# robotseu/ORB_Line_SLAM

Measured on AMD Instinct MI355X. Metric: stereo frames/s extract+match (ORB+LBD), KITTI 1242x375, higher is better.
Workload: dtype u8; 1 GPU; C3: 1242x375 stereo, 2000 ORB + 500 LBD per image, extract + stereo point/line match + f2f LBD match + SearchByBoW vs the previous frame (synthetic k=10 L=6 vocabulary, ComputeBoW included); parallelism=frame-sharded x1, distinct_pairs=512, order=shuffled, scene=default

## Files before the change

orb_line_slam_amd/csrc/api.cpp:

```cpp
#include "ctx.hpp"
#include "staging.hpp"
#include <map>
#include <mutex>

namespace olf {
static thread_local std::string g_err;
void set_error(const std::string& s) { g_err = s; }

int check_device(const olf_ctx* c, const char* who)
{
    int d = -1;
    if (hipGetDevice(&d) != hipSuccess || d != c->device) { set_error(std::string(who) + ": the context belongs to another device than the current one"); return OLF_ERR_INVALID; }
    return OLF_OK;
}

static int check_landscape(const olf_ctx* c, const char* who)
{
    if (c->orb.portrait) {
        set_error(std::string(who) + ": the context's image is portrait (a pyramid level's octree would have round(width / height) == 0 root cells, where the "
                                     "reference divides by zero): no detector runs in it");
        return OLF_ERR_INVALID;
    }
    return OLF_OK;
}
// ... 150 lines not shown
const char* olf_last_error(void) { return g_err.c_str(); }

int olf_device_count(void)
{
    int n = 0;
    if (hipGetDeviceCount(&n) != hipSuccess) return 0;
    return n;
}

int olf_default_params(olf_params* p)
{
    if (!p) return OLF_ERR_INVALID;
    std::memset(p, 0, sizeof(*p));
    p->abi_version = OLF_ABI_VERSION; p->struct_size = (uint32_t)sizeof(olf_params);
    p->orb.nfeatures = 2000; p->orb.scale_factor = 1.2f; p->orb.nlevels = 8; p->orb.ini_th_fast = 20; p->orb.min_th_fast = 7;
    p->line.lsd_nfeatures = 500; p->line.min_line_length = 0.025; p->line.lsd_refine = 0; p->line.lsd_scale = 1.2;
    p->line.lsd_sigma_scale = 0.6; p->line.lsd_quant = 2.0; p->line.lsd_ang_th = 22.5; p->line.lsd_log_eps = 1.0;
    p->line.lsd_density_th = 0.6; p->line.lsd_n_bins = 1024;
    p->line.conv_seed_order = 1;
    p->stereo.fx = 718.856f; p->stereo.bf = 386.1448f; p->stereo.matching_s_ws = 10; p->stereo.line_sim_th = 0.75;
    p->stereo.min_ratio_12_l = 0.9; p->stereo.min_disp = 1.0; p->stereo.line_horiz_th = 0.1; p->stereo.stereo_overlap_th = 0.75;
    p->stereo.ls_min_disp_ratio = 0.7; p->stereo.best_lr_matches = 1;
    return OLF_OK;
}

void olf_ctx_destroy(olf_ctx* c)
{
    if (!c) return;
    if (c->has_tables) angle_tables_release(c->device, c->params.line.conv_libm_float);
    if (c->h_outslab) (void)hipHostFree(c->h_outslab);
    for (void* p : c->allocs) (void)hipFree(p);
    for (void* p : c->scratch) if (p) (void)hipFree(p);
    for (auto& r : c->prof_recs) { (void)hipEventDestroy(r.a); (void)hipEventDestroy(r.b); }
    for (hipEvent_t e : c->prof_pool) (void)hipEventDestroy(e);
    if (c->ev_fork) (void)hipEventDestroy(c->ev_fork);
    if (c->ev_front) (void)hipEventDestroy(c->ev_front);
    if (c->ev_sort) (void)hipEventDestroy(c->ev_sort);
    if (c->ev_lbd) (void)hipEventDestroy(c->ev_lbd);
    if (c->ev_join) (void)hipEventDestroy(c->ev_join);
    if (c->stream2) (void)hipStreamDestroy(c->stream2);
    if (c->stream) (void)hipStreamDestroy(c->stream);
    delete c;
}

int olf_ctx_create(const olf_params* p, int width, int height, int max_images, olf_ctx** out)
{
    if (!p || !out || width < 64 || height < 64 || max_images < 1) { set_error("olf_ctx_create: bad argument"); return OLF_ERR_INVALID; }
    *out = nullptr;
    if (p->abi_version != OLF_ABI_VERSION || p->struct_size != (uint32_t)sizeof(olf_params)) {
        set_error("olf_ctx_create: the parameter block was not initialised by this library's olf_default_params() (abi_version / struct_size differ: "
                  "caller built against another include/orbline_types.h)");
        return OLF_ERR_INVALID;
    }
    int ndev = 0;
    if (hipGetDeviceCount(&ndev) != hipSuccess || ndev < 1) {
        set_error("olf_ctx_create: no HIP device visible (this library has no CPU path)");
        return OLF_ERR_NODEVICE;
    }
    olf_ctx* c = new olf_ctx();
    c->params = *p; c->W = width; c->H = height; c->max_images = max_images;
    int rc = c->orb.build(p->orb, width, height);
    if (rc != OLF_OK) {
        set_error(rc == OLF_ERR_CAPACITY ? "olf_ctx_create: more than 32760 key points on one pyramid level (nfeatures too large for this scale factor / level count)"
                  : (width > kMaxOrbSide || height > kMaxOrbSide) ? "olf_ctx_create: image wider or higher than 4131 pixels (FAST candidates are packed with 12 bits per coordinate)"
                                         : "olf_ctx_create: image size / ORB parameters not supported (every pyramid level needs at least 62 x 62 pixels)");
        delete c; return rc;
    }
    auto fail = [&](int code) { olf_ctx_destroy(c); return code; };
    if (hipGetDevice(&c->device) != hipSuccess) return fail(OLF_ERR_HIP);
    if (hipDeviceGetAttribute(&c->limits.nCU, hipDeviceAttributeMultiprocessorCount, c->device) != hipSuccess || c->limits.nCU <= 0) c->limits.nCU = 64;
    if (hipDeviceGetAttribute(&c->limits.maxLds, hipDeviceAttributeMaxSharedMemoryPerBlock, c->device) != hipSuccess) c->limits.maxLds = 64 * 1024;
    if (hipStreamCreateWithFlags(&c->stream, hipStreamNonBlocking) != hipSuccess) { set_error("hipStreamCreate failed"); return fail(OLF_ERR_HIP); }
    const OrbGeom& g = c->orb.geom;
    const size_t n = (size_t)max_images;
    OrbDeviceBufs& b = c->ob;
    const bool allocTrace = getenv("OLF_ALLOC_TRACE") != nullptr;
#define A(ptr, count) do { if ((rc = dev_alloc(c, &(ptr), (count))) != OLF_OK) return fail(rc); \
                           if (allocTrace) fprintf(stderr, "alloc %-18s %8.3f MB per image\n", #ptr, (double)(count) * sizeof(*(ptr)) / 1e6 / (double)n); } while (0)
    A(b.pyr, n * g.pyrBytes); A(b.blur, n * g.pyrBytes);
    A(b.cells, n * g.totalCells * g.cellCap); A(b.cellCount, n * g.totalCells);
    A(b.cand, n * g.candTotal); A(b.candNode, n * g.candTotal); A(b.candCount, n * g.nlevels);
    if (g.maxNodes > 2048) A(b.octSpill, n * g.nlevels * octree_lds_bytes(g.maxNodes));
    A(b.lvlKp, n * g.kpTotal); A(b.lvlCount, n * g.nlevels); A(b.lvlAngle, n * g.kpTotal);
    A(b.rx, c->orb.rx.size() + 1); A(b.ry, c->orb.ry.size() + 1); A(b.geom, 1); A(b.status, 256);
    A(c->d_sad, ((n + 1) / 2) * g.outCap); A(c->d_bestkey, ((n + 1) / 2) * g.outCap); A(c->d_rowperm, n * g.outCap);
    A(c->d_images, n * width * height);
#undef A
    if (hipMemcpy(b.rx, c->orb.rx.data(), c->orb.rx.size() * sizeof(ResizeCoef), hipMemcpyHostToDevice) != hipSuccess ||
        hipMemcpy(b.ry, c->orb.ry.data(), c->orb.ry.size() * sizeof(ResizeCoef), hipMemcpyHostToDevice) != hipSuccess ||
        hipMemcpy(b.geom, &g, sizeof(OrbGeom), hipMemcpyHostToDevice) != hipSuccess ||
        hipMemset(b.status, 0, 1024) != hipSuccess) {
        set_error("olf_ctx_create: table upload failed");
        return fail(OLF_ERR_HIP);
    }
    rc = c->line.build(p->line, width, height, max_images);
    if (rc != OLF_OK) { set_error("olf_ctx_create: LSD parameters not supported"); return fail(rc); }
    LineGeom& lg = c->line.geom;
    int prLeast = 0, prGreatest = 0;
    (void)hipDeviceGetStreamPriorityRange(&prLeast, &prGreatest);
    if (hipStreamCreateWithPriority(&c->stream2, hipStreamNonBlocking, prLeast) != hipSuccess ||
        hipEventCreateWithFlags(&c->ev_fork, hipEventDisableTiming) != hipSuccess || hipEventCreateWithFlags(&c->ev_front, hipEventDisableTiming) != hipSuccess || hipEventCreateWithFlags(&c->ev_sort, hipEventDisableTiming) != hipSuccess ||
        hipEventCreateWithFlags(&c->ev_lbd, hipEventDisableTiming) != hipSuccess ||
        hipEventCreateWithFlags(&c->ev_join, hipEventDisableTiming) != hipSuccess) { set_error("stream/event creation failed"); return fail(OLF_ERR_HIP); }
    LineDeviceBufs& l = c->lb;
#define A(ptr, count) do { if ((rc = dev_alloc(c, &(ptr), (count))) != OLF_OK) return fail(rc); \
                           if (allocTrace) fprintf(stderr, "alloc %-18s %8.3f MB per image\n", #ptr, (double)(count) * sizeof(*(ptr)) / 1e6 / (double)n); } while (0)
    const bool batchCtx = n > (size_t)kBatchCtxImages;
    const size_t keyWords = lg.wide ? 2 : 1;
    A(l.grad, n * lg.Ps); A(l.keysA, n * lg.Ps * keyWords); A(l.keysB, n * lg.Ps * keyWords);
    if (batchCtx && lg.Ps * 4 >= lg.pitchW * lg.H && lg.Ps * 4 >= lg.pitchS * lg.Hs) { l.lsdBlur = reinterpret_cast<uint8_t*>(l.keysA); l.scaled = reinterpret_cast<uint8_t*>(l.keysB); c->scaled_aliased = true; }
    else { A(l.lsdBlur, n * lg.pitchW * lg.H); A(l.scaled, n * lg.pitchS * lg.Hs); }
    A(l.topBuf, n * (size_t)lsd_seedsort_top_words()); A(l.keyCount, n * 32); A(l.maxN, n * 32); A(l.chunkCnt, n * ((lg.Ps + 4095) / 4096)); A(l.sortHist, n * (size_t)lsd_sort_max_chunks(lg.Ps) * 32); A(l.sortBase, n * 32);
    l.nChunks = lg.regionStride / 32;
    A(l.region, n * (size_t)lg.regionStride); l.ownerImages = (batchCtx || lg.wide) ? 0 : (int)std::min<size_t>(n, kMwMaxImages); A(l.owner, (size_t)l.ownerImages * lg.Ps); A(l.links, n * (size_t)l.nChunks);
    lg.logCap = lg.regionStride / 2;
    lg.spillBlocks = lg.regionStride / 2 >= lg.Ps ? 0 : (int)std::max<size_t>(4, n / 16);
    if (lg.spillBlocks) A(lg.spillArena, (size_t)lg.spillBlocks * 2 * lg.Ps);
    A(lg.spillCtl, 64); A(lg.spillOf, n);
    l.mgImages = (int)std::min<size_t>(n, kMgMaxImages); l.mgStride = lsd_grow_mg_stride(lg.maxRegions);
    A(l.mg, (size_t)l.mgImages * l.mgStride);
    A(l.rawLines, n * lg.maxDetect); A(l.rawCount, n); A(l.regCount, n); A(l.growFmt, n); A(l.lbdBlur, n * lg.pitchW * lg.H); A(l.dxdy, n * lg.pitchD * lg.H);
    A(l.rowSums, n * lg.outCap * 63 * 4); A(l.lbdStarts, n * lg.outCap * 64 * 2); A(l.rx, c->line.rx.size()); A(l.ry, c->line.ry.size()); A(l.geom, 1);
    A(c->d_ldist, ((n + 1) / 2) * lg.outCap * lg.outCap); A(c->d_lm21, ((n + 1) / 2) * lg.outCap);
    if (hipMalloc(&c->d_lprep, stereo_lines_prep_bytes((int)n, lg.outCap)) != hipSuccess) { set_error("hipMalloc failed"); return fail(OLF_ERR_HIP); }
    c->allocs.push_back(c->d_lprep);
    const bool slab = n <= 16;
    if (slab) {
        size_t off = 0;
        for (int k = 0; k < FB_FIELDS; ++k) { c->outslab_off[k] = off; off += (fb_bytes(c, k, n) + 255) & ~(size_t)255; }
        c->outslab_bytes = off;
        A(c->d_outslab, off);
        if (hipHostMalloc(reinterpret_cast<void**>(&c->h_outslab), off, hipHostMallocDefault) != hipSuccess) { set_error("hipHostMalloc failed"); return fail(OLF_ERR_HIP); }
    }
    for (int k = 0; k < FB_FIELDS; ++k) {
        uint8_t* q = nullptr;
        if (slab) q = c->d_outslab + c->outslab_off[k];
        else if ((rc = dev_alloc(c, &q, fb_bytes(c, k, n))) != OLF_OK) return fail(rc);
        fb_set_field(c->d_out, k, q);
        if (allocTrace) fprintf(stderr, "alloc %-18s %8.3f MB per image\n", kFrameFields[k].name, (double)fb_bytes(c, k, n) / 1e6 / (double)n);
    }
#undef A
    l.status = b.status;
    if (hipMemcpy(l.rx, c->line.rx.data(), c->line.rx.size() * sizeof(ResizeCoef), hipMemcpyHostToDevice) != hipSuccess ||
        hipMemcpy(l.ry, c->line.ry.data(), c->line.ry.size() * sizeof(ResizeCoef), hipMemcpyHostToDevice) != hipSuccess ||
        hipMemcpy(l.geom, &lg, sizeof(LineGeom), hipMemcpyHostToDevice) != hipSuccess) { set_error("line table upload failed"); return fail(OLF_ERR_HIP); }
    if ((rc = angle_tables_acquire(c->device, p->line.conv_libm_float, l, c->stream)) != OLF_OK) return fail(rc);
    c->has_tables = true;
    *out = c;
    return OLF_OK;
}

int olf_ctx_synchronize(olf_ctx* c)
{
    if (!c) return OLF_ERR_INVALID;
    OLF_HIP_CHECK(hipStreamSynchronize(c->stream));
    OLF_HIP_CHECK(hipStreamSynchronize(c->stream2));
    c->join_pending = false;
    return check_status(c);
}

int olf_ctx_set_input_event(olf_ctx* c, void* hip_event)
{
    if (!c) return OLF_ERR_INVALID;
    c->input_event = static_cast<hipEvent_t>(hip_event);
    return OLF_OK;
}

int olf_ctx_poll_status(olf_ctx* c)
{
    if (!c) return OLF_ERR_INVALID;
    return check_status(c);
}

// ... 359 lines not shown
```

orb_line_slam_amd/csrc/host_tables.cpp:

```cpp
#include "olf_internal.hpp"
#include "line_internal.hpp"
#include <algorithm>
#include <cmath>
#include <cfenv>

namespace olf {

static inline int cv_round_f(float v) { return (int)lrintf(v); }
static inline int cv_round_d(double v) { return (int)lrint(v); }
static inline int cv_floor(double v) { int i = (int)v; return i - (i > v); }
static inline int cv_ceil(double v) { int i = (int)v; return i + (i < v); }

std::vector<int> gaussian_taps_q8(int n, double sigma, int sum256)
{
    if (sum256) {
        std::vector<double> k(n);
        double s = 0;
        const double scale2X = -0.5 / (sigma * sigma);
        for (int i = 0; i < n; ++i) { const double x = i - (n - 1) * 0.5; k[i] = std::exp(scale2X * x * x); s += k[i]; }
        std::vector<int> q(n);
        double err = 0;
        int sum = 0;
        for (int i = 0; i < n / 2; ++i) {
            const double adj = k[i] / s * 256.0 + err;
            const int v = cv_round_d(adj);
            err = adj - v;
            q[i] = q[n - 1 - i] = v;
            sum += v;
        }
        q[n / 2] = 256 - 2 * sum;
        return q;
    }
    std::vector<float> cf(n);
    double scale2X = -0.5 / (sigma * sigma), sum = 0;
    for (int i = 0; i < n; ++i) {
        double x = i - (n - 1) * 0.5;
        cf[i] = (float)std::exp(scale2X * x * x);
        sum += cf[i];
    }
    sum = 1. / sum;
    std::vector<int> q(n);
    for (int i = 0; i < n; ++i) {
        cf[i] = (float)(cf[i] * sum);
        q[i] = cv_round_d((double)cf[i] * 256.0);
    }
    return q;
}

void resize_axis_coefs(int sn, int dn, double scale, bool clamp_like_x, ResizeCoef* coef)
{
    for (int d = 0; d < dn; ++d) {
        float f = (float)((d + 0.5) * scale - 0.5);
        int s = cv_floor(f);
        f -= s;
        if (clamp_like_x) {
            if (s < 0) { f = 0; s = 0; }
            if (s >= sn - 1) { f = 0; s = sn - 1; }
        }
        int a0 = cv_round_f((1.f - f) * 2048.f), a1 = cv_round_f(f * 2048.f);
        coef[d].ofs = (int16_t)s;
        coef[d].a0 = (int16_t)std::min(std::max(a0, -32768), 32767);
        coef[d].a1 = (int16_t)std::min(std::max(a1, -32768), 32767);
        coef[d].pad = 0;
    }
}

void resize_axis_coefs_exact(int sn, int dn, double scale, ResizeCoef* coef)
{
    for (int d = 0; d < dn; ++d) {
        const double f = scale * (d + 0.5) - 0.5;
        int i = cv_floor(f);
        int a = cv_round_d((f - i) * 256.0);
        if (i < 0) { i = 0; a = 0; }
        if (i >= sn - 1) { i = sn - 1; a = 0; }
        coef[d].ofs = (int16_t)i; coef[d].a0 = (int16_t)(256 - a); coef[d].a1 = (int16_t)a; coef[d].pad = 0;
    }
}

int OrbHostTables::build(const olf_orb_params& p, int W, int H)
{
    const int nlevels = p.nlevels;
    if (nlevels < 1 || nlevels > OLF_MAX_LEVELS || p.nfeatures < 1 || !(p.scale_factor > 1.0f)) return OLF_ERR_INVALID;
    if (W > kMaxOrbSide || H > kMaxOrbSide) return OLF_ERR_INVALID;
    const double scaleFactor = p.scale_factor;
    sf.assign(nlevels, 1.f); sigma2.assign(nlevels, 1.f); inv_sf.resize(nlevels); inv_sigma2.resize(nlevels);
    for (int i = 1; i < nlevels; ++i) {
        sf[i] = (float)(sf[i - 1] * scaleFactor);
        sigma2[i] = sf[i] * sf[i];
    }
    for (int i = 0; i < nlevels; ++i) {
        inv_sf[i] = 1.0f / sf[i];
        inv_sigma2[i] = 1.0f / sigma2[i];
    }
    nPerLevel.resize(nlevels);
    float factor = (float)(1.0f / scaleFactor);
    float nDesired = p.nfeatures * (1 - factor) / (1 - (float)std::pow((double)factor, (double)nlevels));
    int sum = 0;
    for (int l = 0; l < nlevels - 1; ++l) {
        nPerLevel[l] = cv_round_f(nDesired);
        sum += nPerLevel[l];
        nDesired *= factor;
    }
    nPerLevel[nlevels - 1] = std::max(p.nfeatures - sum, 0);

    OrbGeom& g = geom;
    g = OrbGeom();
    g.nlevels = nlevels; g.W = W; g.H = H; g.in_pitch = W;
    g.iniTh = std::min(std::max(p.ini_th_fast, 1), 255);
    g.minTh = std::min(std::max(p.min_th_fast, 1), 255);
    g.minTh = std::min(g.minTh, g.iniTh);
    {
        int v, v0, vmax = cv_floor(kHalfPatch * std::sqrt(2.f) / 2 + 1);
        int vmin = cv_ceil(kHalfPatch * std::sqrt(2.f) / 2);
        const double hp2 = kHalfPatch * kHalfPatch;
        for (v = 0; v <= vmax; ++v) g.umax[v] = cv_round_d(std::sqrt(hp2 - v * v));
        for (v = kHalfPatch, v0 = 0; v >= vmin; --v) {
            while (g.umax[v0] == g.umax[v0 + 1]) ++v0;
            g.umax[v] = v0;
            ++v0;
        }
    }
    std::vector<int> taps = gaussian_taps_q8(7, 2.0, p.conv_gauss_sum256);
    for (int i = 0; i < 7; ++i) g.blurTaps[i] = taps[i];

    rx.clear(); ry.clear();
    int off = 0, cells = 0, cand = 0, kps = 0, cellCap = 1, maxQuota = 1, maxKp = 1;
    for (int l = 0; l < nlevels; ++l) {
        LevelGeom& L = g.lv[l];
        L.w = cv_round_f((float)W * inv_sf[l]);
        L.h = cv_round_f((float)H * inv_sf[l]);
        if (L.w - 2 * kMinBorder < 30 || L.h - 2 * kMinBorder < 30) return OLF_ERR_INVALID;
        L.pitch = (L.w + 63) & ~63;
        L.offset = off;
        off += L.pitch * L.h;
        off = (off + 255) & ~255;
        L.maxBorderX = L.w - kMinBorder; L.maxBorderY = L.h - kMinBorder;
        const float width = (float)(L.maxBorderX - kMinBorder), height = (float)(L.maxBorderY - kMinBorder);
        L.nCols = (int)(width / 30.f); L.nRows = (int)(height / 30.f);
        L.wCell = (int)std::ceil(width / L.nCols); L.hCell = (int)std::ceil(height / L.nRows);
        L.wCellM = (uint32_t)(((1u << 20) + L.wCell - 1) / L.wCell); L.hCellM = (uint32_t)(((1u << 20) + L.hCell - 1) / L.hCell);
        if (L.w >= (1 << 14) || L.h >= (1 << 14) || L.wCell > 64 || L.hCell > 64) { L.wCellM = 0; L.hCellM = 0; }
        L.cellBase = cells;
        cells += L.nCols * L.nRows;
        cellCap = std::max(cellCap, ((L.wCell + 1) / 2) * ((L.hCell + 1) / 2));
        L.quota = nPerLevel[l];
        maxQuota = std::max(maxQuota, L.quota);
        L.nIni = (int)std::round(width / height);
        if (L.nIni < 1) { portrait = true; L.nIni = 1; }
        L.hX = width / L.nIni;
        L.scale = sf[l]; L.inv_scale = inv_sf[l];
        L.patch_size = (int)(31 * sf[l]);
        L.kpBase = kps; L.kpCap = std::max(L.quota + 8, 4 * L.nIni + 4); kps += L.kpCap;
        maxKp = std::max(maxKp, L.kpCap);
        if (l > 0) {
            const LevelGeom& P = g.lv[l - 1];
            L.resizeTabX = (int)rx.size(); L.resizeTabY = (int)ry.size();
            rx.resize(rx.size() + L.w); ry.resize(ry.size() + L.h);
            double inv_x = (double)L.w / P.w, inv_y = (double)L.h / P.h;
            resize_axis_coefs(P.w, L.w, 1. / inv_x, true, &rx[L.resizeTabX]);
            resize_axis_coefs(P.h, L.h, 1. / inv_y, false, &ry[L.resizeTabY]);
            L.resizeTiled = resize_tiled_fits(&rx[L.resizeTabX], &ry[L.resizeTabY], P.w, P.h, L.w, L.h) ? 1 : 0;
            if (L.resizeTiled && resize_strip_fits(&rx[L.resizeTabX], P.w, L.w)) L.resizeTiled |= 2;
        }
    }
    g.pyrBytes = off;
    g.totalCells = cells;
    g.cellCap = cellCap;
    if (cellCap > 1024) return OLF_ERR_CAPACITY;
    for (int l = 0; l < nlevels; ++l) {
        LevelGeom& L = g.lv[l];
        long cap = (long)L.nCols * L.nRows * cellCap;
        L.candCap = (int)std::min<long>(cap, 65535);
        L.candBase = cand;
        cand += (L.candCap + 63) & ~63;
    }
    g.candTotal = cand;
    g.kpTotal = kps;
    g.outCap = kps;
    int mn = 64;
    while (mn < maxKp) mn <<= 1;
    g.maxNodes = mn;
    if (mn > 32768) return OLF_ERR_CAPACITY;
    return OLF_OK;
}

int LineHostTables::build(const olf_line_params& p, int W, int H, int max_images)
{
    LineGeom& g = geom;
    g = LineGeom();
    if (p.lsd_refine < 0 || p.lsd_refine > 2) return OLF_ERR_INVALID;
    if (p.conv_seed_order != 0 && p.conv_seed_order != 1) return OLF_ERR_INVALID;
    if (p.conv_libm_float != 0 && p.conv_libm_float != 1) return OLF_ERR_INVALID;
    if (!(p.lsd_scale > 0) || p.lsd_n_bins < 2 || p.lsd_n_bins > (1 << 24) || !(p.lsd_ang_th > 0 && p.lsd_ang_th < 180)) return OLF_ERR_INVALID;
    const double kPI = 3.1415926535897932384626433832795;
    g.W = W; g.H = H; g.pitchW = (W + 63) & ~63; g.pitchD = (W + 3) & ~3;
    g.scale = p.lsd_scale;
    g.Ws = cv_round_d(W * p.lsd_scale); g.Hs = cv_round_d(H * p.lsd_scale);
    g.pitchS = (g.Ws + 63) & ~63;
    g.Ps = g.Ws * g.Hs;
    {
        int k = 0; while ((1 << k) < g.Ws) ++k;
        const int p = std::max(32, 22 + k);
// ... 87 lines not shown
```

orb_line_slam_amd/csrc/olf_internal.hpp:

```cpp
#pragma once
#include <hip/hip_runtime.h>
#include <stdint.h>
#include <string>
#include <vector>
#include "../../include/orbline_types.h"
#include "device_math.hpp"

#define OLF_HIP_CHECK(expr)                                                                 \
    do {                                                                                    \
        hipError_t _e = (expr);                                                             \
        if (_e != hipSuccess) {                                                             \
            olf::set_error(std::string(#expr) + ": " + hipGetErrorString(_e));              \
            return OLF_ERR_HIP;                                                             \
        }                                                                                   \
    } while (0)

#define OLF_TRY(expr)                  \
    do {                               \
        int _rc = (expr);              \
        if (_rc != OLF_OK) return _rc; \
    } while (0)

struct olf_ctx;

// ... 50 lines not shown
}
OLF_HD void csr_row(const int* __restrict__ offs, int n, int k, int& b, int& e) { const int last = offs[n]; csr_clamp(offs, k, last > 0 ? last : 0, b, e); }

OLF_HD int live_item(int v, int n_items, const uint8_t* __restrict__ bad, int* __restrict__ status, int bit)
{
    if (v >= n_items) { status_raise(status, bit); return -1; }
    return v < 0 || bad[v] ? -1 : v;
}

#ifdef __HIPCC__
__device__ __forceinline__ bool pair_in_batch(int f1, int f2, int n_frames) { return f1 >= 0 && f1 < n_frames && f2 >= 0 && f2 < n_frames && f1 != f2; }

__device__ __forceinline__ int wave_sum_i32(int v)
{
    v += __builtin_amdgcn_mov_dpp(v, 0xB1, 0xf, 0xf, true);
    v += __builtin_amdgcn_mov_dpp(v, 0x4E, 0xf, 0xf, true);
    v += __builtin_amdgcn_mov_dpp(v, 0x141, 0xf, 0xf, true);
    v += __builtin_amdgcn_mov_dpp(v, 0x140, 0xf, 0xf, true);
    return __builtin_amdgcn_readlane(v, 0) + __builtin_amdgcn_readlane(v, 16) + __builtin_amdgcn_readlane(v, 32) + __builtin_amdgcn_readlane(v, 48);
}

__device__ __forceinline__ int wave_min_i32(int v)
{
    v = min(v, __builtin_amdgcn_update_dpp(v, v, 0xB1, 0xf, 0xf, false));
    v = min(v, __builtin_amdgcn_update_dpp(v, v, 0x4E, 0xf, 0xf, false));
    v = min(v, __builtin_amdgcn_update_dpp(v, v, 0x141, 0xf, 0xf, false));
    v = min(v, __builtin_amdgcn_update_dpp(v, v, 0x140, 0xf, 0xf, false));
    return min(min(__builtin_amdgcn_readlane(v, 0), __builtin_amdgcn_readlane(v, 16)), min(__builtin_amdgcn_readlane(v, 32), __builtin_amdgcn_readlane(v, 48)));
}
__device__ __forceinline__ unsigned long long wave_vote(bool p) { return __builtin_amdgcn_ballot_w64(p); }
__device__ __forceinline__ int wave_rank_below(unsigned long long m) { return (int)__builtin_amdgcn_mbcnt_hi((unsigned)(m >> 32), __builtin_amdgcn_mbcnt_lo((unsigned)m, 0u)); }
__device__ __forceinline__ bool wave_bit(unsigned long long m) { return __builtin_amdgcn_inverse_ballot_w64(m); }
#endif

constexpr int kEdge = 19;
constexpr int kMinBorder = 16;
constexpr int kHalfPatch = 15;
constexpr int kMaxOrbSide = 4095 + 2 * kMinBorder + 4;
static_assert(kMaxOrbSide == 4131, "olf_ctx_create's message and include/orbline.h state this limit");

struct LevelGeom {
    int w, h, pitch;
    int offset;
    int maxBorderX, maxBorderY;
    int nCols, nRows, wCell, hCell;
    uint32_t wCellM, hCellM;
    int cellBase;
    int quota;
    int nIni;
    float hX;
    float scale;
    float inv_scale;
    int patch_size;
    int candBase;
    int candCap;
    int kpBase, kpCap;
    int resizeTabX, resizeTabY;
    int resizeTiled;
};

struct ResizeCoef { int16_t ofs; int16_t a0; int16_t a1; int16_t pad; };

struct OrbGeom {
    int nlevels;
    int W, H, in_pitch;
    int pyrBytes;
    int totalCells;
    int cellCap;
    int candTotal;
    int kpTotal;
    int outCap;
    int iniTh, minTh;
    int maxNodes;
    LevelGeom lv[OLF_MAX_LEVELS];
    int umax[16];
    int blurTaps[7];
};

struct OrbHostTables {
    std::vector<float> sf, inv_sf, sigma2, inv_sigma2;
    std::vector<int> nPerLevel;
    OrbGeom geom;
    std::vector<ResizeCoef> rx, ry;
    bool portrait = false;
    int build(const olf_orb_params& p, int W, int H);
};

std::vector<int> gaussian_taps_q8(int n, double sigma, int sum256 = 0);
void resize_axis_coefs(int sn, int dn, double scale, bool clamp_like_x, ResizeCoef* coef);

struct OrbDeviceBufs {
    uint8_t* pyr = nullptr;
    uint8_t* blur = nullptr;
    uint32_t* cells = nullptr;
    int* cellCount = nullptr;
    uint32_t* cand = nullptr;
    uint16_t* candNode = nullptr;
    int* candCount = nullptr;
    uint32_t* lvlKp = nullptr;
    int* lvlCount = nullptr;
    float* lvlAngle = nullptr;
    ResizeCoef* rx = nullptr;
    ResizeCoef* ry = nullptr;
    OrbGeom* geom = nullptr;
    int* status = nullptr;
    unsigned char* octSpill = nullptr;
};

int launch_orb_pyramid(const OrbGeom& g, const OrbDeviceBufs& b, const uint8_t* d_in, int n_images, hipStream_t s);
int launch_orb_fast(const OrbGeom& g, const OrbDeviceBufs& b, int n_images, hipStream_t s);
int launch_orb_octree(const OrbGeom& g, const OrbDeviceBufs& b, int n_images, hipStream_t s);
size_t octree_lds_bytes(int M);
int launch_orb_blur(const OrbGeom& g, const OrbDeviceBufs& b, int n_images, hipStream_t s);
int launch_orb_describe(const OrbGeom& g, const OrbDeviceBufs& b, int n_images, olf_keypoint* d_kps, uint8_t* d_desc,
                        int* d_counts, int out_cap, hipStream_t s);

struct Taps7 { int t[7]; };
int launch_sep7(const uint8_t* src, size_t srcImgStride, int srcPitch, uint8_t* dst, size_t dstImgStride, int dstPitch, int W, int H,
                const int* taps7, int n_images, hipStream_t s);
int launch_sep_wide(const uint8_t* src, size_t srcImgStride, int srcPitch, uint8_t* dst, size_t dstImgStride, int dstPitch, int W, int H,
                    const int* taps, int r, int n_images, hipStream_t s);

bool resize_tiled_fits(const ResizeCoef* rx, const ResizeCoef* ry, int sw, int sh, int dw, int dh);
bool resize_strip_fits(const ResizeCoef* rx, int sw, int dw, int ncols = 4);
int launch_resize_tiled(const uint8_t* src, size_t srcImgStride, int srcPitch, int sw, int sh, uint8_t* dst, size_t dstImgStride, int dstPitch,
                        int dw, int dh, const ResizeCoef* d_rx, const ResizeCoef* d_ry, int n_images, hipStream_t s, bool strip = false);

int launch_cvt_gray(const uint8_t* src, uint8_t* dst, int w, int h, int code, int n_images, hipStream_t s);
int launch_init_rectify_map(const double* ir9, const double* k8, double fx, double fy, double u0, double v0, int w, int h, float* d_map1, float* d_map2,
                            hipStream_t s);
int launch_remap_linear(const uint8_t* src, int sw, int sh, const float* mapx, const float* mapy, int dw, int dh, uint8_t* dst, int n_images,
                        hipStream_t s);

int launch_stereo_points(const OrbGeom& g, const OrbDeviceBufs& b, int n_pairs, const olf_keypoint* d_kps, const uint8_t* d_desc,
                         const int* d_counts, int cap, float mbf, float fx, float* d_uRight, float* d_depth, int* d_sad, int* d_bestKey,
                         unsigned* d_perm, hipStream_t s);
int launch_match_bf(const uint8_t* dA, const int* nA, int strideA, int aStep, const uint8_t* dB, const int* nB, int strideB, int bStep,
                    int n_sets, float nnr, int best_lr, int* ws, int* m12, hipStream_t s);
int launch_knn2(const uint8_t* dA, const int* nA, int strideA, const uint8_t* dB, const int* nB, int strideB, int n_sets, int* idx0,
                int* dist0, int* dist1, hipStream_t s);
int launch_knn2_indexed(const uint8_t* q, const int* rank_entry, const int* qidx, const int* qbase, const int* nQ, const int* tile_prefix, int n_sets,
                        int max_tiles, const uint8_t* t, const int* nT, int strideT, int tStep, int tCap, int* idx0, int* dist0, int* dist1, hipStream_t s);
int launch_match_candidates(const uint8_t* q, int nQ, const uint8_t* t, int nT, const int* offs, const int* cand, uint16_t* out, hipStream_t s);
int launch_distinctive(const uint8_t* desc, const int* offs, int n_points, int* best, hipStream_t s);
int launch_hamming_matrix(const uint8_t* a, int nA, const uint8_t* b, int nB, uint16_t* out, hipStream_t s);


inline bool grid_scales(float minX, float maxX, float minY, float maxY, float* wInv, float* hInv)
{
    if (!(maxX > minX) || !(maxY > minY)) return false;
    *wInv = static_cast<float>(OLF_GRID_COLS) / (maxX - minX);
    *hInv = static_cast<float>(OLF_GRID_ROWS) / (maxY - minY);
    return true;
}
int launch_assign_grid(const olf_keypoint* d_kps, size_t frame_stride, const int* d_counts, int count_stride, int n_fixed, int n_limit, float minX,
                       float minY, float wInv, float hInv, int n_frames, int* d_cell_offsets, int* d_cell_index, size_t index_stride, hipStream_t s);
int launch_features_in_area(const olf_keypoint* d_keys, const int* d_cell_offsets, const int* d_cell_index, float minX, float minY, float wInv, float hInv,
                            int n_queries, const olf_area_query* d_queries, int* d_cand_offsets, int* d_cand_idx, int cand_capacity, int* d_status,
                            hipStream_t s);
bool grid_is_valid(const int32_t* cell_offsets, const int32_t* cell_index, int n);

int launch_kfdb_tables(const int* d_qoff, const int* d_qids, const double* d_qvals, int n_queries, const int* d_beg, const int* d_len, const int* d_ids,
                       const double* d_vals, int n_slots, int* d_common, int* d_first, double* d_score, hipStream_t s);
int launch_bow_score_pairs(const int* d_pairs, int n_pairs, const int* a_beg, const int* a_len, int n_a, const int* a_ids, const double* a_vals,
                           const int* b_beg, const int* b_len, int n_b, const int* b_ids, const double* b_vals, double* d_score, hipStream_t s);

}
```

orb_line_slam_amd/csrc/orb_describe.hip:

```cpp
#include "olf_internal.hpp"
#include "device_math.hpp"

namespace olf {

__constant__ __attribute__((aligned(16))) int8_t c_pattern[1024] = {
#include "orb_pattern_31.inc"
};

constexpr int DESC_KPW = 1;

__global__ __launch_bounds__(256) void k_describe(const OrbGeom* __restrict__ gp, const uint8_t* __restrict__ pyr,
                                                  const uint8_t* __restrict__ blur, const uint32_t* __restrict__ lvlKp,
                                                  const int* __restrict__ lvlCount, olf_keypoint* __restrict__ kps,
                                                  uint8_t* __restrict__ desc, int* __restrict__ counts, int out_cap,
                                                  int* __restrict__ status)
{
    constexpr int PR = 18, PW = 2 * PR + 1, PDW = 10;
    __shared__ float4 s_patf[256];
    __shared__ uint32_t s_w0[256], s_w1[256];
    __shared__ uint32_t s_patch[4][PW * PDW];
    const OrbGeom& g = *gp;
    const int img = blockIdx.y, lane = threadIdx.x & 63, wv = threadIdx.x >> 6;
    {
        const uint32_t pw = reinterpret_cast<const uint32_t*>(c_pattern)[threadIdx.x];
        s_patf[threadIdx.x] = make_float4((float)(int8_t)(pw & 0xff), (float)(int8_t)((pw >> 8) & 0xff), (float)(int8_t)((pw >> 16) & 0xff), (float)(int8_t)(pw >> 24));
    }
    {
        const int r = threadIdx.x >> 3, j = threadIdx.x & 7, v = r - kHalfPatch;
        uint32_t w0 = 0, w1 = 0;
        if (r <= 2 * kHalfPatch) {
            const int d = g.umax[v < 0 ? -v : v];
#pragma unroll
            for (int b = 0; b < 4; ++b) {
                const int u = 4 * j + b - 16;
                if (u >= -d && u <= d) { w0 |= 1u << (8 * b); w1 |= (uint32_t)(u + 16) << (8 * b); }
            }
        }
        s_w0[threadIdx.x] = w0; s_w1[threadIdx.x] = w1;
    }
    __syncthreads();
    const int nlevels = g.nlevels, kpTotal = g.kpTotal;
    const int* lc = lvlCount + img * nlevels;
    if (blockIdx.x == 0 && threadIdx.x == 0) {
        int tot = 0;
        for (int l = 0; l < nlevels; ++l) tot += lc[l];
        if (tot > out_cap) { atomicOr(status, 4); tot = out_cap; }
        counts[img] = tot;
    }
    const int nbx = (int)gridDim.x, per = nbx >> 3;
    const int vblock = ((int)blockIdx.x < per * 8) ? ((int)blockIdx.x & 7) * per + ((int)blockIdx.x >> 3) : (int)blockIdx.x;
    const int r6 = lane / PDW, c10 = lane - r6 * PDW;
    uint32_t* patch = s_patch[wv];
#pragma unroll 1
    for (int q = 0; q < DESC_KPW; ++q) {
        const int slot = (vblock * 4 + wv) * DESC_KPW + q;
        if (slot >= kpTotal) break;
        const uint32_t p = lvlKp[(size_t)img * kpTotal + slot];
        const bool lv_lane = lane < nlevels;
        const int base_l = lv_lane ? g.lv[lane].kpBase : 0x7fffffff, cnt_l = lv_lane ? lc[lane] : 0;
        const int level = (int)__popcll(wave_vote(lv_lane && lane > 0 && slot >= base_l));
        const int i = slot - __builtin_amdgcn_readlane(base_l, level);
        if (i >= __builtin_amdgcn_readlane(cnt_l, level)) continue;
        const int outIdx = i + wave_sum_i32(lane < level ? cnt_l : 0);
        if (outIdx >= out_cap) continue;
        const LevelGeom& L = g.lv[level];
        const int cx = (int)(p >> 20) + kMinBorder, cy = (int)((p >> 8) & 0xfff) + kMinBorder, score = (int)(p & 0xff);
        const int pitch = L.pitch;

        const uint8_t* bl = blur + (size_t)img * g.pyrBytes + L.offset;
        const int x0 = (cx - PR) & ~3, xs = cx - x0;
        uint32_t stg[(PW + 5) / 6];
        {
            const int xo = min(x0 + 4 * c10, pitch - 4);
            const uint32_t stBase = (uint32_t)((cy - PR + r6) * pitch + xo);
#pragma unroll
            for (int k = 0; k < (PW + 5) / 6; ++k) {
                stg[k] = 0u;
                if (lane < 60 && 6 * k + r6 < PW) stg[k] = *reinterpret_cast<const uint32_t*>(bl + (stBase + (uint32_t)(6 * k * pitch)));
            }
        }

        const uint8_t* im = pyr + (size_t)img * g.pyrBytes + L.offset;
        int m10 = 0, m01 = 0, sI = 0;
        const uint32_t icBase = (uint32_t)((cy - kHalfPatch + (lane >> 3)) * pitch + cx - 16 + 4 * (lane & 7));
#pragma unroll
        for (int pass = 0; pass < 4; ++pass) {
            if (pass * 64 + lane < (2 * kHalfPatch + 1) * 8) {
                uint32_t I;
                __builtin_memcpy(&I, im + (icBase + (uint32_t)(pass * 8 * pitch)), 4);
                const int rs = (int)__builtin_amdgcn_udot4(I, s_w0[pass * 64 + lane], 0u, false);
                m10 = (int)__builtin_amdgcn_udot4(I, s_w1[pass * 64 + lane], (uint32_t)m10, false);
                sI += rs;
                m01 += (pass * 8 + (lane >> 3) - kHalfPatch) * rs;
            }
        }
        m10 -= 16 * sI;
        m10 = wave_sum_i32(m10);
        m01 = wave_sum_i32(m01);
        const float angle = dev_fastAtan2((float)m01, (float)m10);

        const float factorPI = (float)(3.1415926535897932384626433832795 / 180.f);
        const float rad = __fmul_rn(angle, factorPI);
        const float a = glibc_cosf(rad), b = glibc_sinf(rad);
        __builtin_amdgcn_wave_barrier();
#pragma unroll
        for (int k = 0; k < (PW + 5) / 6; ++k)
            if (lane < 60 && 6 * k + r6 < PW) patch[60 * k + lane] = stg[k];
        __builtin_amdgcn_wave_barrier();
        const uint8_t* pb = reinterpret_cast<const uint8_t*>(patch) + PR * (PDW * 4) + xs;
        unsigned long long bits[4];
#pragma unroll
        for (int j = 0; j < 4; ++j) {
            const float4 pt = s_patf[j * 64 + lane];
            const int r0 = __float2int_rn(__fadd_rn(__fmul_rn(pt.x, b), __fmul_rn(pt.y, a)));
            const int c0 = __float2int_rn(__fsub_rn(__fmul_rn(pt.x, a), __fmul_rn(pt.y, b)));
            const int r1 = __float2int_rn(__fadd_rn(__fmul_rn(pt.z, b), __fmul_rn(pt.w, a)));
            const int c1 = __float2int_rn(__fsub_rn(__fmul_rn(pt.z, a), __fmul_rn(pt.w, b)));
            const int t0 = pb[r0 * (PDW * 4) + c0], t1 = pb[r1 * (PDW * 4) + c1];
            bits[j] = wave_vote(t0 < t1);
        }
        if (lane == 0) {
            unsigned long long* d = reinterpret_cast<unsigned long long*>(desc + ((size_t)img * out_cap + outIdx) * OLF_DESC_BYTES);
            d[0] = bits[0]; d[1] = bits[1]; d[2] = bits[2]; d[3] = bits[3];
            olf_keypoint k;
            k.x = (float)cx; k.y = (float)cy;
            if (level != 0) { k.x = __fmul_rn(k.x, L.scale); k.y = __fmul_rn(k.y, L.scale); }
            k.size = (float)L.patch_size; k.angle = angle; k.response = (float)score; k.octave = level; k.class_id = -1;
            kps[(size_t)img * out_cap + outIdx] = k;
        }
    }
}

int launch_orb_describe(const OrbGeom& g, const OrbDeviceBufs& b, int n_images, olf_keypoint* d_kps, uint8_t* d_desc,
                        int* d_counts, int out_cap, hipStream_t s)
{
    hipLaunchKernelGGL(k_describe, dim3((g.kpTotal + 4 * DESC_KPW - 1) / (4 * DESC_KPW), n_images), dim3(256), 0, s, b.geom, b.pyr, b.blur, b.lvlKp, b.lvlCount,
                       d_kps, d_desc, d_counts, out_cap, b.status);
    OLF_HIP_CHECK(hipGetLastError());
    return OLF_OK;
}

}
```

Measured before the change: 15010 stereo frames/s.

## Pipeline ORB describe over compacted keypoint runs with precomputed device tables

The describe kernel now gives each wave a run of 4 compacted output keypoints instead of one padded slot. It software-pipelines the global loads for the moment disc and the blurred patch of the next keypoint behind the computation of the current one. The pattern and moment weight tables are built once on the host and uploaded, replacing per-block construction from constant memory and the umax table. The grid shrinks by about 4x, and float-to-int rounding uses a magic-constant add trick. This cuts launch and padding waste and hides memory latency, at the cost of more registers and more complex indexing.

```diff
diff --git a/orb_line_slam_amd/csrc/api.cpp b/orb_line_slam_amd/csrc/api.cpp
--- a/orb_line_slam_amd/csrc/api.cpp
+++ b/orb_line_slam_amd/csrc/api.cpp
@@ -256,13 +256,14 @@
     A(b.cand, n * g.candTotal); A(b.candNode, n * g.candTotal); A(b.candCount, n * g.nlevels);
     if (g.maxNodes > 2048) A(b.octSpill, n * g.nlevels * octree_lds_bytes(g.maxNodes));
     A(b.lvlKp, n * g.kpTotal); A(b.lvlCount, n * g.nlevels); A(b.lvlAngle, n * g.kpTotal);
-    A(b.rx, c->orb.rx.size() + 1); A(b.ry, c->orb.ry.size() + 1); A(b.geom, 1); A(b.status, 256);
+    A(b.rx, c->orb.rx.size() + 1); A(b.ry, c->orb.ry.size() + 1); A(b.geom, 1); A(b.describeTab, kDescribeTabWords); A(b.status, 256);
     A(c->d_sad, ((n + 1) / 2) * g.outCap); A(c->d_bestkey, ((n + 1) / 2) * g.outCap); A(c->d_rowperm, n * g.outCap);
     A(c->d_images, n * width * height);
 #undef A
     if (hipMemcpy(b.rx, c->orb.rx.data(), c->orb.rx.size() * sizeof(ResizeCoef), hipMemcpyHostToDevice) != hipSuccess ||
         hipMemcpy(b.ry, c->orb.ry.data(), c->orb.ry.size() * sizeof(ResizeCoef), hipMemcpyHostToDevice) != hipSuccess ||
         hipMemcpy(b.geom, &g, sizeof(OrbGeom), hipMemcpyHostToDevice) != hipSuccess ||
+        hipMemcpy(b.describeTab, c->orb.describeTab.data(), kDescribeTabWords * sizeof(uint32_t), hipMemcpyHostToDevice) != hipSuccess ||
         hipMemset(b.status, 0, 1024) != hipSuccess) {
         set_error("olf_ctx_create: table upload failed");
         return fail(OLF_ERR_HIP);
diff --git a/orb_line_slam_amd/csrc/host_tables.cpp b/orb_line_slam_amd/csrc/host_tables.cpp
--- a/orb_line_slam_amd/csrc/host_tables.cpp
+++ b/orb_line_slam_amd/csrc/host_tables.cpp
@@ -3,6 +3,7 @@
 #include <algorithm>
 #include <cmath>
 #include <cfenv>
+#include <cstring>
 
 namespace olf {
 
@@ -118,6 +119,23 @@
             while (g.umax[v0] == g.umax[v0 + 1]) ++v0;
             g.umax[v] = v0;
             ++v0;
+        }
+    }
+    {
+        static const int8_t pattern[1024] = {
+#include "orb_pattern_31.inc"
+        };
+        describeTab.assign(kDescribeTabWords, 0u);
+        for (int i = 0; i < 1024; ++i) {
+            const float f = (float)pattern[i];
+            std::memcpy(&describeTab[i], &f, 4);
+        }
+        for (int t = 0; t < (2 * kHalfPatch + 1) * 8; ++t) {
+            const int v = t / 8 - kHalfPatch, j = t % 8, d = g.umax[v < 0 ? -v : v];
+            for (int b = 0; b < 4; ++b) {
+                const int u = 4 * j + b - 16;
+                if (u >= -d && u <= d) { describeTab[1024 + t] |= 1u << (8 * b); describeTab[1280 + t] |= (uint32_t)(u + 16) << (8 * b); }
+            }
         }
     }
     std::vector<int> taps = gaussian_taps_q8(7, 2.0, p.conv_gauss_sum256);
diff --git a/orb_line_slam_amd/csrc/olf_internal.hpp b/orb_line_slam_amd/csrc/olf_internal.hpp
--- a/orb_line_slam_amd/csrc/olf_internal.hpp
+++ b/orb_line_slam_amd/csrc/olf_internal.hpp
@@ -156,12 +156,15 @@
     std::vector<int> nPerLevel;
     OrbGeom geom;
     std::vector<ResizeCoef> rx, ry;
+    std::vector<uint32_t> describeTab;
     bool portrait = false;
     int build(const olf_orb_params& p, int W, int H);
 };
 
 std::vector<int> gaussian_taps_q8(int n, double sigma, int sum256 = 0);
 void resize_axis_coefs(int sn, int dn, double scale, bool clamp_like_x, ResizeCoef* coef);
+
+constexpr int kDescribeTabWords = 1024 + 256 + 256;
 
 struct OrbDeviceBufs {
     uint8_t* pyr = nullptr;
@@ -177,6 +180,7 @@
     ResizeCoef* rx = nullptr;
     ResizeCoef* ry = nullptr;
     OrbGeom* geom = nullptr;
+    uint32_t* describeTab = nullptr;
     int* status = nullptr;
     unsigned char* octSpill = nullptr;
 };
diff --git a/orb_line_slam_amd/csrc/orb_describe.hip b/orb_line_slam_amd/csrc/orb_describe.hip
--- a/orb_line_slam_amd/csrc/orb_describe.hip
+++ b/orb_line_slam_amd/csrc/orb_describe.hip
@@ -3,139 +3,180 @@
 
 namespace olf {
 
-__constant__ __attribute__((aligned(16))) int8_t c_pattern[1024] = {
-#include "orb_pattern_31.inc"
-};
+constexpr int DESC_RUN = 4;
 
-constexpr int DESC_KPW = 1;
+constexpr int DESC_PR = 18, DESC_PW = 2 * DESC_PR + 1, DESC_PDW = 10;
+constexpr int DESC_NSTG = (DESC_PW + 5) / 6;
 
-__global__ __launch_bounds__(256) void k_describe(const OrbGeom* __restrict__ gp, const uint8_t* __restrict__ pyr,
+__device__ __forceinline__ size_t scalar_u64(size_t v)
+{
+    const unsigned lo = (unsigned)__builtin_amdgcn_readfirstlane((int)(unsigned)v), hi = (unsigned)__builtin_amdgcn_readfirstlane((int)(unsigned)(v >> 32));
+    return ((size_t)hi << 32) | lo;
+}
+
+__global__ __launch_bounds__(256, 8) void k_describe(const OrbGeom* __restrict__ gp, const uint32_t* __restrict__ tab, const uint8_t* __restrict__ pyr,
                                                   const uint8_t* __restrict__ blur, const uint32_t* __restrict__ lvlKp,
                                                   const int* __restrict__ lvlCount, olf_keypoint* __restrict__ kps,
                                                   uint8_t* __restrict__ desc, int* __restrict__ counts, int out_cap,
-                                                  int* __restrict__ status)
+                                                  int* __restrict__ status, int nlevels, int kpTotal, int pyrBytes)
 {
-    constexpr int PR = 18, PW = 2 * PR + 1, PDW = 10;
+    constexpr int PR = DESC_PR, PW = DESC_PW, PDW = DESC_PDW;
     __shared__ float4 s_patf[256];
     __shared__ uint32_t s_w0[256], s_w1[256];
     __shared__ uint32_t s_patch[4][PW * PDW];
-    const OrbGeom& g = *gp;
     const int img = blockIdx.y, lane = threadIdx.x & 63, wv = threadIdx.x >> 6;
-    {
-        const uint32_t pw = reinterpret_cast<const uint32_t*>(c_pattern)[threadIdx.x];
-        s_patf[threadIdx.x] = make_float4((float)(int8_t)(pw & 0xff), (float)(int8_t)((pw >> 8) & 0xff), (float)(int8_t)((pw >> 16) & 0xff), (float)(int8_t)(pw >> 24));
-    }
-    {
-        const int r = threadIdx.x >> 3, j = threadIdx.x & 7, v = r - kHalfPatch;
-        uint32_t w0 = 0, w1 = 0;
-        if (r <= 2 * kHalfPatch) {
-            const int d = g.umax[v < 0 ? -v : v];
-#pragma unroll
-            for (int b = 0; b < 4; ++b) {
-                const int u = 4 * j + b - 16;
-                if (u >= -d && u <= d) { w0 |= 1u << (8 * b); w1 |= (uint32_t)(u + 16) << (8 * b); }
-            }
-        }
-        s_w0[threadIdx.x] = w0; s_w1[threadIdx.x] = w1;
-    }
-    __syncthreads();
-    const int nlevels = g.nlevels, kpTotal = g.kpTotal;
-    const int* lc = lvlCount + img * nlevels;
-    if (blockIdx.x == 0 && threadIdx.x == 0) {
-        int tot = 0;
-        for (int l = 0; l < nlevels; ++l) tot += lc[l];
-        if (tot > out_cap) { atomicOr(status, 4); tot = out_cap; }
-        counts[img] = tot;
-    }
+    const float4 tpat = reinterpret_cast<const float4*>(tab)[threadIdx.x];
+    const uint32_t tw0 = tab[1024 + threadIdx.x], tw1 = tab[1280 + threadIdx.x];
+    const bool lv_lane = lane < nlevels;
+    const LevelGeom& Ll = gp->lv[lv_lane ? lane : 0];
+    const int cnt_m = lvlCount[img * nlevels + (lv_lane ? lane : 0)], cnt_l = lv_lane ? cnt_m : 0;
+    const int base_l = Ll.kpBase, geo_l = Ll.offset | (Ll.pitch >> 6);
     const int nbx = (int)gridDim.x, per = nbx >> 3;
     const int vblock = ((int)blockIdx.x < per * 8) ? ((int)blockIdx.x & 7) * per + ((int)blockIdx.x >> 3) : (int)blockIdx.x;
+    const int j0 = (vblock * 4 + wv) * DESC_RUN, j = j0 + lane;
+    int tot = 0, lvl_q = 0, slot_q = 0;
+    for (int l = 0; l < nlevels; ++l) {
+        const int c = __builtin_amdgcn_readlane(cnt_l, l), b = __builtin_amdgcn_readlane(base_l, l);
+        if (j >= tot && j < tot + c) { lvl_q = l; slot_q = b + (j - tot); }
+        tot += c;
+    }
+    if (blockIdx.x == 0 && threadIdx.x == 0) {
+        if (tot > out_cap) atomicOr(status, 4);
+        counts[img] = min(tot, out_cap);
+    }
+    const int nrun = min(DESC_RUN, min(tot, out_cap) - j0);
+    const uint32_t p_q = lvlKp[(size_t)img * kpTotal + slot_q];
+    s_patf[threadIdx.x] = tpat; s_w0[threadIdx.x] = tw0; s_w1[threadIdx.x] = tw1;
+    __syncthreads();
+    if (nrun <= 0) return;
     const int r6 = lane / PDW, c10 = lane - r6 * PDW;
     uint32_t* patch = s_patch[wv];
-#pragma unroll 1
-    for (int q = 0; q < DESC_KPW; ++q) {
-        const int slot = (vblock * 4 + wv) * DESC_KPW + q;
-        if (slot >= kpTotal) break;
-        const uint32_t p = lvlKp[(size_t)img * kpTotal + slot];
-        const bool lv_lane = lane < nlevels;
-        const int base_l = lv_lane ? g.lv[lane].kpBase : 0x7fffffff, cnt_l = lv_lane ? lc[lane] : 0;
-        const int level = (int)__popcll(wave_vote(lv_lane && lane > 0 && slot >= base_l));
-        const int i = slot - __builtin_amdgcn_readlane(base_l, level);
-        if (i >= __builtin_amdgcn_readlane(cnt_l, level)) continue;
-        const int outIdx = i + wave_sum_i32(lane < level ? cnt_l : 0);
-        if (outIdx >= out_cap) continue;
-        const LevelGeom& L = g.lv[level];
-        const int cx = (int)(p >> 20) + kMinBorder, cy = (int)((p >> 8) & 0xfff) + kMinBorder, score = (int)(p & 0xff);
-        const int pitch = L.pitch;
+    const size_t imgOff = scalar_u64((size_t)img * pyrBytes);
+    const uint8_t* blImg = blur + imgOff;
+    const uint8_t* pyImg = pyr + imgOff;
 
-        const uint8_t* bl = blur + (size_t)img * g.pyrBytes + L.offset;
-        const int x0 = (cx - PR) & ~3, xs = cx - x0;
-        uint32_t stg[(PW + 5) / 6];
-        {
-            const int xo = min(x0 + 4 * c10, pitch - 4);
-            const uint32_t stBase = (uint32_t)((cy - PR + r6) * pitch + xo);
+    struct Kp { int cx, cy, score, level, pitch, offset; };
+    auto key_point = [&](int q) {
+        const uint32_t p = (uint32_t)__builtin_amdgcn_readlane((int)p_q, q);
+        const int level = __builtin_amdgcn_readlane(lvl_q, q), geo = __builtin_amdgcn_readlane(geo_l, level);
+        return Kp{(int)(p >> 20) + kMinBorder, (int)((p >> 8) & 0xfff) + kMinBorder, (int)(p & 0xff), level, (geo & 0xff) << 6, geo & ~0xff};
+    };
+
+    auto request_disc = [&](int q, uint32_t (&ic)[4]) {
+        const Kp k = key_point(q);
+        const uint8_t* im = pyImg + k.offset;
+        const uint32_t icBase = (uint32_t)((k.cy - kHalfPatch + (lane >> 3)) * k.pitch + k.cx - 16 + 4 * (lane & 7));
+        const uint32_t icLast = (uint32_t)((k.cy - kHalfPatch + 24 + min(lane >> 3, 6)) * k.pitch + k.cx - 16 + 4 * (lane & 7));
 #pragma unroll
-            for (int k = 0; k < (PW + 5) / 6; ++k) {
-                stg[k] = 0u;
-                if (lane < 60 && 6 * k + r6 < PW) stg[k] = *reinterpret_cast<const uint32_t*>(bl + (stBase + (uint32_t)(6 * k * pitch)));
-            }
-        }
-
-        const uint8_t* im = pyr + (size_t)img * g.pyrBytes + L.offset;
+        for (int pass = 0; pass < 4; ++pass)
+            __builtin_memcpy(&ic[pass], im + (pass < 3 ? icBase + (uint32_t)(pass * 8 * k.pitch) : icLast), 4);
+    };
+    int m10_q = 0, m01_q = 0;
+    auto moments = [&](int q, const uint32_t (&ic)[4]) {
         int m10 = 0, m01 = 0, sI = 0;
-        const uint32_t icBase = (uint32_t)((cy - kHalfPatch + (lane >> 3)) * pitch + cx - 16 + 4 * (lane & 7));
 #pragma unroll
         for (int pass = 0; pass < 4; ++pass) {
-            if (pass * 64 + lane < (2 * kHalfPatch + 1) * 8) {
-                uint32_t I;
-                __builtin_memcpy(&I, im + (icBase + (uint32_t)(pass * 8 * pitch)), 4);
-                const int rs = (int)__builtin_amdgcn_udot4(I, s_w0[pass * 64 + lane], 0u, false);
-                m10 = (int)__builtin_amdgcn_udot4(I, s_w1[pass * 64 + lane], (uint32_t)m10, false);
-                sI += rs;
-                m01 += (pass * 8 + (lane >> 3) - kHalfPatch) * rs;
-            }
+            const uint32_t I = ic[pass];
+            const int rs = (int)__builtin_amdgcn_udot4(I, s_w0[pass * 64 + lane], 0u, false);
+            m10 = (int)__builtin_amdgcn_udot4(I, s_w1[pass * 64 + lane], (uint32_t)m10, false);
+            sI += rs;
+            m01 += (pass * 8 + (lane >> 3) - kHalfPatch) * rs;
         }
         m10 -= 16 * sI;
         m10 = wave_sum_i32(m10);
         m01 = wave_sum_i32(m01);
-        const float angle = dev_fastAtan2((float)m01, (float)m10);
+        if (lane == q) { m10_q = m10; m01_q = m01; }
+    };
+    {
+        uint32_t icA[4];
+        request_disc(0, icA);
+#pragma unroll 1
+        for (int q = 0; q + 1 < nrun; ++q) {
+            uint32_t icB[4];
+            request_disc(q + 1, icB);
+            __builtin_amdgcn_sched_barrier(0);
+            moments(q, icA);
+#pragma unroll
+            for (int pass = 0; pass < 4; ++pass) icA[pass] = icB[pass];
+        }
+        moments(nrun - 1, icA);
+    }
 
-        const float factorPI = (float)(3.1415926535897932384626433832795 / 180.f);
-        const float rad = __fmul_rn(angle, factorPI);
-        const float a = glibc_cosf(rad), b = glibc_sinf(rad);
+    auto request_patch = [&](int q, uint32_t (&stg)[DESC_NSTG]) {
+        const Kp k = key_point(q);
+        const uint8_t* bl = blImg + k.offset;
+        const int x0 = (k.cx - PR) & ~3;
+        const int xo = min(x0 + 4 * c10, k.pitch - 4);
+        const uint32_t stBase = (uint32_t)((k.cy - PR + r6) * k.pitch + xo);
+#pragma unroll
+        for (int s = 0; s < DESC_NSTG; ++s) {
+            const uint32_t o = 6 * s + 6 < PW ? stBase + (uint32_t)(6 * s * k.pitch) : (uint32_t)((k.cy - PR + PW - 1) * k.pitch + xo);
+            stg[s] = *reinterpret_cast<const uint32_t*>(bl + o);
+        }
+    };
+    uint32_t stgA[DESC_NSTG];
+    request_patch(0, stgA);
+
+    const float angle_q = dev_fastAtan2((float)m01_q, (float)m10_q);
+    const float factorPI = (float)(3.1415926535897932384626433832795 / 180.f);
+    const float rad_q = __fmul_rn(angle_q, factorPI);
+    const float a_q = glibc_cosf(rad_q), b_q = glibc_sinf(rad_q);
+
+    auto describe = [&](int q, const uint32_t (&stg)[DESC_NSTG]) {
+        const Kp k = key_point(q);
+        const int outIdx = j0 + q;
+        const float angle = __builtin_bit_cast(float, __builtin_amdgcn_readlane(__builtin_bit_cast(int, angle_q), q));
+        const float a = __builtin_bit_cast(float, __builtin_amdgcn_readlane(__builtin_bit_cast(int, a_q), q));
+        const float b = __builtin_bit_cast(float, __builtin_amdgcn_readlane(__builtin_bit_cast(int, b_q), q));
         __builtin_amdgcn_wave_barrier();
 #pragma unroll
-        for (int k = 0; k < (PW + 5) / 6; ++k)
-            if (lane < 60 && 6 * k + r6 < PW) patch[60 * k + lane] = stg[k];
+        for (int s = 0; s < DESC_NSTG; ++s)
+            if (lane < 60 && 6 * s + r6 < PW) patch[60 * s + lane] = stg[s];
         __builtin_amdgcn_wave_barrier();
-        const uint8_t* pb = reinterpret_cast<const uint8_t*>(patch) + PR * (PDW * 4) + xs;
+        const float kRound = 12582912.f;
+        const uint32_t xs = (uint32_t)(k.cx - ((k.cx - PR) & ~3));
+        const uint32_t pb0 = (uint32_t)(PR * (PDW * 4)) + xs - (0x400000u * (uint32_t)(PDW * 4) + 0x4B400000u);
+        const uint8_t* pbytes = reinterpret_cast<const uint8_t*>(patch);
+        auto at = [&](float r, float c) {
+            const int ri = __builtin_bit_cast(int, __fadd_rn(r, kRound)), ci = __builtin_bit_cast(int, __fadd_rn(c, kRound));
+            return pbytes[(uint32_t)(__mul24(ri, PDW * 4) + ci) + pb0];
+        };
         unsigned long long bits[4];
 #pragma unroll
-        for (int j = 0; j < 4; ++j) {
-            const float4 pt = s_patf[j * 64 + lane];
-            const int r0 = __float2int_rn(__fadd_rn(__fmul_rn(pt.x, b), __fmul_rn(pt.y, a)));
-            const int c0 = __float2int_rn(__fsub_rn(__fmul_rn(pt.x, a), __fmul_rn(pt.y, b)));
-            const int r1 = __float2int_rn(__fadd_rn(__fmul_rn(pt.z, b), __fmul_rn(pt.w, a)));
-            const int c1 = __float2int_rn(__fsub_rn(__fmul_rn(pt.z, a), __fmul_rn(pt.w, b)));
-            const int t0 = pb[r0 * (PDW * 4) + c0], t1 = pb[r1 * (PDW * 4) + c1];
-            bits[j] = wave_vote(t0 < t1);
+        for (int t = 0; t < 4; ++t) {
+            const float4 pt = s_patf[t * 64 + lane];
+            const int t0 = at(__fadd_rn(__fmul_rn(pt.x, b), __fmul_rn(pt.y, a)), __fsub_rn(__fmul_rn(pt.x, a), __fmul_rn(pt.y, b)));
+            const int t1 = at(__fadd_rn(__fmul_rn(pt.z, b), __fmul_rn(pt.w, a)), __fsub_rn(__fmul_rn(pt.z, a), __fmul_rn(pt.w, b)));
+            bits[t] = wave_vote(t0 < t1);
         }
         if (lane == 0) {
             unsigned long long* d = reinterpret_cast<unsigned long long*>(desc + ((size_t)img * out_cap + outIdx) * OLF_DESC_BYTES);
             d[0] = bits[0]; d[1] = bits[1]; d[2] = bits[2]; d[3] = bits[3];
-            olf_keypoint k;
-            k.x = (float)cx; k.y = (float)cy;
-            if (level != 0) { k.x = __fmul_rn(k.x, L.scale); k.y = __fmul_rn(k.y, L.scale); }
-            k.size = (float)L.patch_size; k.angle = angle; k.response = (float)score; k.octave = level; k.class_id = -1;
-            kps[(size_t)img * out_cap + outIdx] = k;
+            olf_keypoint r;
+            r.x = (float)k.cx; r.y = (float)k.cy;
+            const LevelGeom& L = gp->lv[k.level];
+            if (k.level != 0) { r.x = __fmul_rn(r.x, L.scale); r.y = __fmul_rn(r.y, L.scale); }
+            r.size = (float)L.patch_size; r.angle = angle; r.response = (float)k.score; r.octave = k.level; r.class_id = -1;
+            kps[(size_t)img * out_cap + outIdx] = r;
         }
+    };
+#pragma unroll 1
+    for (int q = 0; q + 1 < nrun; ++q) {
+        uint32_t stgB[DESC_NSTG];
+        request_patch(q + 1, stgB);
+        __builtin_amdgcn_sched_barrier(0);
+        describe(q, stgA);
+#pragma unroll
+        for (int s = 0; s < DESC_NSTG; ++s) stgA[s] = stgB[s];
     }
+    describe(nrun - 1, stgA);
 }
 
 int launch_orb_describe(const OrbGeom& g, const OrbDeviceBufs& b, int n_images, olf_keypoint* d_kps, uint8_t* d_desc,
                         int* d_counts, int out_cap, hipStream_t s)
 {
-    hipLaunchKernelGGL(k_describe, dim3((g.kpTotal + 4 * DESC_KPW - 1) / (4 * DESC_KPW), n_images), dim3(256), 0, s, b.geom, b.pyr, b.blur, b.lvlKp, b.lvlCount,
-                       d_kps, d_desc, d_counts, out_cap, b.status);
+    hipLaunchKernelGGL(k_describe, dim3((g.kpTotal + 4 * DESC_RUN - 1) / (4 * DESC_RUN), n_images), dim3(256), 0, s, b.geom, b.describeTab, b.pyr, b.blur,
+                       b.lvlKp, b.lvlCount, d_kps, d_desc, d_counts, out_cap, b.status, g.nlevels, g.kpTotal, g.pyrBytes);
     OLF_HIP_CHECK(hipGetLastError());
     return OLF_OK;
 }
```

Measured after the change: 15110 stereo frames/s (median of 6 runs). About the same (+0.7%).
